# caterer-z-t/GRiD

Measured on AMD Instinct MI355X. Metric: samples/sec end-to-end steps 4–7 (50k×3M bins); k-NN distance HBM GB/s vs peak, higher is better.
Workload: dtype f64 (statistics) + bf16-MFMA exact-integer (k-NN)

## Files before the change

grid_amd/_abi.py:

```python
from __future__ import annotations

import ctypes as C
import os
import sys
from pathlib import Path

import numpy as np

_HERE = Path(__file__).resolve().parent
LIB_PATH = Path(os.environ.get("GRID_AMD_LIB", _HERE / "_lib" / "libgridhip.so"))

GRID_OK, GRID_EINVAL, GRID_EHIP, GRID_EZERODIV, GRID_EUNSUPPORTED, GRID_ERANGE = range(6)
MISSING = -(2 ** 31)
ZQ_NAN = -(2 ** 31)
ZQ_NEG0 = -(2 ** 31) + 1
ZQ16_NAN, ZQ16_NEG0, ZQ16_ESC = -32768, -32767, -32766
BLOCK = 8192
KBW = 32
SEG_K1 = 16
SEL_STATE = 16
SEL_NVALID, SEL_RLOC, SEL_RTOT, SEL_NV, SEL_RUSE, SEL_ERR = 0, 1, 2, 3, 4, 5
SEL_THR, SEL_V0, SEL_SMIN, SEL_SMAX = 8, 9, 12, 13

_i64, _i32, _f64, _vp = C.c_int64, C.c_int32, C.c_double, C.c_void_p
# ... 122 lines not shown
    "grid_md_parse_map": [_vp, _vp, _vp, _vp, _i64, _vp, _vp, _vp, _vp, _vp, _vp, _i64, _vp, _i64, _vp, _i64, _vp,
                          _vp, _vp],
    "grid_md_parse_ref_general": [_vp, _vp, _vp, _vp, _i64, _vp, _vp, _vp, _vp, _vp, _i64, _vp, _vp, _vp, _vp,
                                  C.POINTER(_i64)],
    "grid_md_parse_map_general": [_vp, _vp, _vp, _vp, _i64, _vp, _vp, _vp, _vp, _vp, _vp, _i64, _vp, _i64, _vp, _i64,
                                  _vp, _vp, _vp],
    "grid_fill_i32": [_vp, _vp, _i64, _i32],
    "grid_md_finish": [_vp, _vp, _i64, _i64, _i64, _vp, _i32, _f64, _f64, _vp, _vp, _vp, _vp, _vp, C.POINTER(_i64)],
    "grid_md_gather": [_vp, _vp, _i64, _i64, _i64, _vp, _vp, _vp, _vp, _i64, _vp, _vp, _vp],
    "grid_ctx_own_stream_cumask": [_vp, _vp, _i32],
    "grid_ctx_stream": [_vp, C.POINTER(_vp)],
    "grid_knn_seg_pack": [_vp, _vp, _i64, _i64, _i64, _vp],
    "grid_knn_seg_tiles_pack": [_vp, _vp, _i64, _i64, _i64, _i64, _vp],
    "grid_knn_seg_rows_fill": [_vp, _vp, _i64, _vp, _i64, _i64, _i64, _vp, _i64],
    "grid_md_popsum": [_vp, _vp, _i64, _i64, _vp, _i32, _vp, _vp],
    "grid_md_popvalid": [_vp, _vp, _vp, _i64, _f64, _f64, _vp],
    "grid_md_rowstats": [_vp, _vp, _i64, _i64, _i64, _vp, _vp, _vp, _vp, C.POINTER(_i64)],
    "grid_md_pack_shards": [_vp, _vp, _i64, _i64, _vp, _vp, _vp, _i32, _vp, _i32, _vp],
    "grid_gz_parts_new": [C.POINTER(_vp)],
    "grid_gz_parts_header": [_vp, _i64, _i64, _vp, _vp, _i32, _i32],
    "grid_gz_parts_rows": [_vp, _i64, _i64, _i64, C.c_char_p, _vp, _vp, _i64, _i32, _i32],
    "grid_gz_parts_rows_dev": [_vp, _vp, _i64, _i64, _i64, C.c_char_p, _vp, _vp, _i64, _i32, _i64],
    "grid_gz_parts_size": [_vp, C.POINTER(_i64)],
    "grid_gz_parts_write": [_vp, C.c_char_p, _i64, _i32],
    "grid_gz_parts_free": [_vp],
    "grid_ntext_count": [_vp, _vp, _vp, _vp, _i64, _vp, _vp, _vp, _i64, _vp, _vp, _vp, _vp, _vp, _vp],
    "grid_ntext_parse": [_vp, _vp, _vp, _vp, _vp, _i64, _vp, _vp, _vp, _i64, _i64, _vp, _i64, _vp, _vp, _vp],
    "grid_ntext_prefix": [_vp, _vp, _i64, _vp, _i64, _vp],
    "grid_ntext_parse_host": [_vp, _i64, _i64, _i64, _i64, _vp, _i64, _vp, _i64, C.POINTER(_i32), C.POINTER(_i64)],
    "grid_ntext_rows_host": [_vp, _i64, _vp, _i64, C.POINTER(_i64), _vp, _vp],
    "grid_ntext_index_open": [C.c_char_p, _i32, C.POINTER(_vp), C.POINTER(_i64), C.POINTER(_i64), C.POINTER(_i64)],
    "grid_ntext_index_fetch": [_vp, _vp, _vp, _vp, _vp, _vp, _vp],
    "grid_ntext_index_free": [_vp],
}
EXPORTS = tuple(_SIGS) + ("grid_last_error", "grid_build_info")


class GridNativeError(RuntimeError):

    def __init__(self, msg, code=None):
        super().__init__(msg)
        self.code = code


_lib = None


def load():
    global _lib
    if _lib is not None:
        return _lib
    if not LIB_PATH.exists():
        raise GridNativeError(f"{LIB_PATH} not built: run `python -c 'import __graft_entry__ as g; g.build()'` "
                              "or `make -C grid_amd/csrc`")
    lib = C.CDLL(str(LIB_PATH), mode=C.RTLD_GLOBAL)
    try:
        for name, args in _SIGS.items():
            f = getattr(lib, name)
            f.argtypes = args
            f.restype = C.c_int
        lib.grid_last_error.argtypes = []
        lib.grid_last_error.restype = C.c_char_p
        info = _build_info(lib)
    except AttributeError as e:
        raise GridNativeError(f"{LIB_PATH} lacks an entry point this package binds ({e}): rebuild with "
                              "`make -C grid_amd/csrc`") from None
    files = info.get("src_files")
    if files and (_CSRC / "Makefile").exists():
        named = sorted(n for n in files.split() if not n.startswith(".."))
        if named != _HASHED:
            raise GridNativeError(f"{LIB_PATH} hashed other source files ({' '.join(named)}) than this tree "
                                  f"lists: rebuild with `make -C grid_amd/csrc`")
    want = source_sha256(files.split() if files else None)
    if want is not None and info.get("src_sha256") != want:
        raise GridNativeError(f"{LIB_PATH} was built from other sources (library {info.get('src_sha256')}, "
                              f"tree {want}): rebuild with `make -C grid_amd/csrc`")
    _lib = lib
    return lib


_CSRC = _HERE / "csrc"
_HASHED = sorted(["core.hip", "normalize.hip", "knn.hip", "dipcn_phase.hip", "synth.hip", "depth16.hip",
                  "inflate.hip", "mosdepth_dev.hip", "gzwrite.hip", "ntext_dev.hip", "ingest.cpp", "textio.cpp",
                  "hapnbr.cpp", "common.hpp", "synth_model.hpp", "inflate_core.hpp", "ntext_core.hpp", "fastgz.hpp"])


def source_sha256(names=None):
    import hashlib
    if names is not None:
        files = [_CSRC / f for f in names]
    else:
        files = [_CSRC / f for f in _HASHED] + [_HERE.parent / "include" / "grid_abi.h"]
    if not all(f.exists() for f in files):
        return None
    h = hashlib.sha256()
    for f in files:
        h.update(f.read_bytes())
    return h.hexdigest()


def _build_info(lib):
    import json
    lib.grid_build_info.argtypes = [C.c_char_p, C.c_int64]
    lib.grid_build_info.restype = C.c_int
    buf = C.create_string_buffer(512)
    lib.grid_build_info(buf, 512)
    return json.loads(buf.value.decode())


def build_info():
    return _build_info(load())


def check(rc: int, what: str = ""):
    if rc == GRID_OK:
        return
    msg = load().grid_last_error().decode(errors="replace")
    if rc == GRID_EZERODIV:
        raise ZeroDivisionError(msg or "float division by zero")
    raise GridNativeError(f"{what}: {msg} (code {rc})", rc)


def call(name: str, *args):
    check(getattr(load(), name)(*args), name)


def ptr(a) -> int:
    if a is None:
        return None
    if isinstance(a, np.ndarray):
        if not a.flags.c_contiguous:
            raise ValueError("array must be C-contiguous")
        return a.ctypes.data
    if isinstance(a, DevBuf):
        return a.ptr
    if hasattr(a, "data_ptr"):
        return a.data_ptr()
    return int(a)


class PinnedBuf:

    def __init__(self, nbytes: int):
        h = _vp()
        call("grid_host_alloc", int(nbytes), C.byref(h))
        self.ptr, self.nbytes = h.value, int(nbytes)
        self.array = np.ctypeslib.as_array((C.c_uint8 * self.nbytes).from_address(self.ptr))

    def free(self):
        if self.ptr:
            self.array = None
            load().grid_host_free(self.ptr)
            self.ptr = 0

    def __del__(self):
        try:
            self.free()
        except Exception:
            pass


class Device:

    def __init__(self, device: int = 0, stream=None):
        lib = load()
        self.index = device
        h = _vp()
# ... 572 lines not shown
```

grid_amd/csrc/mosdepth_dev.hip:

```cpp
#include "common.hpp"

#include <hipcub/hipcub.hpp>

#include <algorithm>

namespace {

constexpr int CH = 16384, SEG = 64, PTH = CH / SEG, MAXLINE = 256;

struct MdOpts {
  const char *prefix;
  int npre;
  int has_window;
  int64_t wstart, wend;
  int nmask;
  const char *mnames;
  const int32_t *mname_off;
  const int64_t *mkb_off;
  const int64_t *mkb;
};

template <class P>
__device__ __forceinline__ bool md_masked(const MdOpts &o, P c, int clen, int64_t s, int64_t e) {
  if (o.nmask == 0) return false;
  const bool has = clen >= 3 && c[0] == 'c' && c[1] == 'h' && c[2] == 'r';
  const int nlen = has ? clen : clen + 3;
  for (int k = 0; k < o.nmask; k++) {
    const int a = o.mname_off[k], b = o.mname_off[k + 1];
    if (b - a != nlen) continue;
    bool eq = true;
    for (int t = 0; t < nlen && eq; t++) {
      const char want = o.mnames[a + t];
      const char got = has ? (char)c[t] : (t < 3 ? "chr"[t] : (char)c[t - 3]);
      eq = want == got;
    }
    if (!eq) continue;
    const int64_t lo = s >= 0 ? s / 1000 : -((-s + 999) / 1000);
    const int64_t hi = e >= 0 ? e / 1000 : -((-e + 999) / 1000);
    if (hi < lo) return false;
    int64_t l = o.mkb_off[k], r = o.mkb_off[k + 1];
    while (l < r) {
      const int64_t m = (l + r) >> 1;
      if (o.mkb[m] < lo) l = m + 1;
      else r = m;
    }
    return l < o.mkb_off[k + 1] && o.mkb[l] <= hi;
  }
  return false;
}

__device__ __forceinline__ uint32_t nl_bits(uint32_t w) {
  const uint32_t x = w ^ 0x0A0A0A0Au;
  return ~(((x & 0x7F7F7F7Fu) + 0x7F7F7F7Fu) | x | 0x7F7F7F7Fu);
}

__global__ __launch_bounds__(256) void k_md_count(const uint8_t *__restrict__ text, const int64_t *__restrict__ toff,
                                                  const int64_t *__restrict__ tlen, const int32_t *__restrict__ cfile,
                                                  const int64_t *__restrict__ cstart, int32_t *__restrict__ cnl,
                                                  int32_t *__restrict__ flags, const int32_t *__restrict__ fst) {
  const int c = blockIdx.x, f = cfile[c];
  if (fst && fst[f]) return;
  const int64_t a = cstart[c], b = min(tlen[f], a + CH);
  const uint8_t *t = text + toff[f];
  int n = 0, hi = 0;
  for (int64_t i = a + threadIdx.x * 16; i < b; i += 256 * 16) {
    if (i + 16 <= b) {
      const uint4 v = *reinterpret_cast<const uint4 *>(t + i);
      n += __builtin_popcount(nl_bits(v.x)) + __builtin_popcount(nl_bits(v.y)) + __builtin_popcount(nl_bits(v.z)) +
           __builtin_popcount(nl_bits(v.w));
      hi |= ((v.x | v.y | v.z | v.w) & 0x80808080u) != 0;
    } else {
      for (int64_t j = i; j < b; j++) {
        n += t[j] == '\n';
        hi |= t[j] >= 0x80;
      }
    }
  }
  for (int o = 32; o > 0; o >>= 1) {
    n += __shfl_xor(n, o, 64);
    hi |= __shfl_xor(hi, o, 64);
  }
  __shared__ int s_n[4], s_hi[4];
  if ((threadIdx.x & 63) == 0) {
// ... 7 lines not shown
  }
}

__global__ __launch_bounds__(256) void k_md_scan(const int32_t *__restrict__ cfirst, const int32_t *__restrict__ cnl,
                                                 int64_t *__restrict__ cline0, int nfiles) {
  __shared__ int64_t s_w[4];
  const int f = blockIdx.x, tid = threadIdx.x, lane = tid & 63, wv = tid >> 6;
  if (f >= nfiles) return;
  const int c0 = cfirst[f], c1 = cfirst[f + 1];
  int64_t base = 0;
  for (int r = c0; r < c1; r += 256) {
    const int c = r + tid;
    const int64_t v = c < c1 ? cnl[c] : 0;
    int64_t incl = v;
#pragma unroll
    for (int d = 1; d < 64; d <<= 1) {
      const int64_t y = __shfl_up(incl, d, 64);
      if (lane >= d) incl += y;
    }
    if (lane == 63) s_w[wv] = incl;
    __syncthreads();
    int64_t before = base;
    for (int w = 0; w < wv; w++) before += s_w[w];
    if (c < c1) cline0[c] = before + incl - v;
    base += s_w[0] + s_w[1] + s_w[2] + s_w[3];
    __syncthreads();
  }
}

template <class P>
__device__ __forceinline__ bool md_line(P p, int len, int &clen, int64_t &s, int64_t &e, int64_t &q) {
  int i = 0;
  while (i < len && (unsigned)(p[i] - 0x21) < 0x5e) i++;
  if (i == 0 || i == len || p[i] != '\t') return false;
  clen = i++;
  int64_t v[2];
  for (int k = 0; k < 2; k++) {
    const int d = i;
    int64_t x = 0;
    while (i < len && (unsigned)(p[i] - '0') < 10) x = x * 10 + (p[i++] - '0');
    if (i == d || i - d > 18 || i == len || p[i] != '\t') return false;
    v[k] = x;
    i++;
  }
  const int d = i;
  int64_t ip = 0;
  while (i < len && (unsigned)(p[i] - '0') < 10) ip = ip * 10 + (p[i++] - '0');
  if (i == d || i - d > 15) return false;
  int64_t fp = 0;
  if (i < len) {
    if (p[i] != '.') return false;
    i++;
    const int f0 = i;
    while (i < len && (unsigned)(p[i] - '0') < 10) fp = fp * 10 + (p[i++] - '0');
    if (i != len || i - f0 > 2) return false;
    if (i - f0 == 1) fp *= 10;
  }
  q = ip * 100 + fp;
  if (q > 2147483647LL) return false;
  s = v[0];
  e = v[1];
  return true;
}

struct Key2 {
  int64_t s, e;
};

__device__ __forceinline__ bool key_lt(int64_t as, int64_t ae, const Key2 &b) {
  return as < b.s || (as == b.s && ae < b.e);
}

__device__ __forceinline__ uint32_t nl_mask16(const uint4 v) {
  const uint32_t w[4] = {v.x, v.y, v.z, v.w};
  uint32_t m = 0;
#pragma unroll
  for (int k = 0; k < 4; k++) {
    const uint32_t z = nl_bits(w[k]);
    m |= (((z >> 7) & 1u) | ((z >> 14) & 2u) | ((z >> 21) & 4u) | ((z >> 28) & 8u)) << (4 * k);
  }
  return m;
}

__device__ __forceinline__ int md_phys(int i) { return i + 4 * ((i + 48) >> 6); }
struct PadText {
  const uint8_t *t;
  int i0;
  __device__ __forceinline__ uint8_t operator[](int k) const { return t[md_phys(i0 + k)]; }
};

constexpr int64_t MD_TAG_MAXLINE = 0x7fffffffLL - 3;
__device__ __forceinline__ int32_t md_tag(int64_t idx) { return (int32_t)(GRID_MISSING + 1 + (int32_t)idx); }

#ifndef GRID_MDPARSE_WPE
#define GRID_MDPARSE_WPE 8
#endif
#ifndef GRID_MDPARSE_G
#define GRID_MDPARSE_G 3
#endif
template <int MODE>
__global__ __launch_bounds__(PTH) __attribute__((amdgpu_waves_per_eu(GRID_MDPARSE_WPE))) void k_md_parse(const uint8_t *__restrict__ text, const int64_t *__restrict__ toff,
                                                  const int64_t *__restrict__ tlen,
                                                  const int32_t *__restrict__ cfile,
                                                  const int64_t *__restrict__ cstart,
                                                  const int64_t *__restrict__ cline0, MdOpts o,
                                                  int32_t *__restrict__ flags,
                                                  uint8_t *__restrict__ ref_kept, Key2 *__restrict__ ref_keys,
                                                  int64_t ref_cap,
                                                  const Key2 *__restrict__ K, int64_t nK,
                                                  const int32_t *__restrict__ ref_kidx, int64_t ref_nlines,
                                                  int32_t *__restrict__ Q, int64_t ldq,
                                                  const int32_t *__restrict__ qrow,
                                                  unsigned long long *__restrict__ kept,
                                                  const int32_t *__restrict__ fst) {
  constexpr int HALO = 16, SPAN = HALO + CH + MAXLINE + 16;
  static_assert(HALO == 16 && SEG == 64, "md_phys: block t + 1 = segment t");
  __shared__ __attribute__((aligned(16))) uint8_t s_t[SPAN + 4 * (SPAN / 64 + 2)];
  __shared__ int s_wsum[PTH / 64];
  const int c = blockIdx.x, f = cfile[c], tid = threadIdx.x;
  if (fst && fst[f]) return;
  const int64_t L = tlen[f], a = cstart[c], b = min(L, a + CH);
  const uint8_t *t = text + toff[f];
  {
    const int64_t lo = a - HALO, hi = min(L, b + MAXLINE);
    constexpr int NW = SPAN / 16, G = GRID_MDPARSE_G;
    for (int k0 = 0; k0 * PTH < NW; k0 += G) {
      uint4 v[G];
#pragma unroll
      for (int k = 0; k < G; k++) {
        const int w = tid + (k0 + k) * PTH;
        const int64_t p = lo + 16 * (int64_t)w;
        v[k] = make_uint4(0, 0, 0, 0);
        if (w < NW && p >= 0 && p + 16 <= hi) v[k] = *reinterpret_cast<const uint4 *>(t + p);
      }
#pragma unroll
      for (int k = 0; k < G; k++) {
        const int w = tid + (k0 + k) * PTH;
        const int64_t p = lo + 16 * (int64_t)w;
        if (w >= NW) continue;
        if (p >= 0 && p + 16 > hi && p < hi) {
          uint8_t q[16];
          for (int j = 0; j < 16; j++) q[j] = p + j < hi ? t[p + j] : 0;
          v[k] = *reinterpret_cast<const uint4 *>(q);
        }
        uint32_t *d = reinterpret_cast<uint32_t *>(s_t + md_phys(16 * w));
        d[0] = v[k].x;
        d[1] = v[k].y;
        d[2] = v[k].z;
        d[3] = v[k].w;
      }
    }
  }
  __syncthreads();
  const int64_t s0 = a + (int64_t)tid * SEG, s1 = min(b, s0 + SEG);
  const int nw = s1 > s0 ? (int)((s1 - s0 + 15) / 16) : 0;
  const uint32_t *seg = reinterpret_cast<const uint32_t *>(s_t + md_phys(HALO + tid * SEG));
  auto mask = [&](int k) {
    uint32_t mk = nl_mask16(make_uint4(seg[4 * k], seg[4 * k + 1], seg[4 * k + 2], seg[4 * k + 3]));
    const int64_t rest = s1 - (s0 + 16 * k);
    if (rest < 16) mk &= (1u << rest) - 1u;
    return mk;
  };
  int nl = 0;
  for (int k = 0; k < nw; k++) nl += __builtin_popcount(mask(k));
  int incl = nl;
#pragma unroll
  for (int d = 1; d < 64; d <<= 1) {
    const int y = __shfl_up(incl, d, 64);
    if ((tid & 63) >= d) incl += y;
  }
  if ((tid & 63) == 63) s_wsum[tid >> 6] = incl;
  __syncthreads();
  int before = incl - nl;
  for (int w = 0; w < (tid >> 6); w++) before += s_wsum[w];
  const int64_t idx0 = cline0[c] + before;
  int bad = 0;
  unsigned long long nkept = 0;
  auto line = [&](int64_t x, int len, int64_t idx) {
    const PadText p{s_t, (int)(HALO + (x - a))};
    if (o.npre != 0) {
      if (len < o.npre) return;
      for (int k = 0; k < o.npre; k++)
        if (p[k] != (uint8_t)o.prefix[k]) return;
    }
    int clen;
    int64_t s, e, q;
    if (!md_line(p, len, clen, s, e, q)) {
      bad |= GRID_MD_EXOTIC;
      return;
    }
    if (!((MODE == 0 || q > 0) && (!o.has_window || (e >= o.wstart && s <= o.wend)) &&
          !md_masked(o, p, clen, s, e)))
      return;
    if (MODE == 0) {
      if (idx < ref_cap) {
        ref_kept[idx] = 1;
        ref_keys[idx] = Key2{s, e};
      } else {
        bad |= GRID_MD_NOTINK;
      }
    } else {
      int64_t j = idx < ref_nlines ? ref_kidx[idx] : -1;
      if (j < 0 || K[j].s != s || K[j].e != e) {
        int64_t l = 0, r = nK;
        while (l < r) {
          const int64_t mid = (l + r) >> 1;
          if (K[mid].s < s || (K[mid].s == s && K[mid].e < e)) l = mid + 1;
          else r = mid;
        }
        j = (l < nK && K[l].s == s && K[l].e == e) ? l : -1;
      }
      if (j < 0) {
        bad |= GRID_MD_NOTINK;
      } else if (MODE == 1) {
        Q[(int64_t)qrow[f] * ldq + j] = (int32_t)q;
        nkept++;
      } else if (idx > MD_TAG_MAXLINE) {
        bad |= GRID_MD_LINES;
      } else {
        int32_t *cell = Q + (int64_t)qrow[f] * ldq + j;
        const int32_t tag = md_tag(idx);
        if (MODE == 2) {
          atomicMax(cell, tag);
        } else if (*cell == tag) {
          *cell = (int32_t)q;
          nkept++;
        }
      }
    }
  };
  if (s1 > s0) {
    int64_t cur = (s0 == 0 || s_t[md_phys((int)(HALO + (s0 - a) - 1))] == '\n') ? s0 : -1;
    int64_t idx = idx0;
    for (int k = 0; k < nw; k++) {
      uint32_t mk = mask(k);
      while (mk) {
        const int64_t y = s0 + 16 * k + __builtin_ctz(mk);
        mk &= mk - 1;
        if (cur >= 0) {
          const int64_t len = y - cur;
          if (len > MAXLINE) bad |= GRID_MD_EXOTIC;
          else line(cur, (int)len, idx);
        }
        idx++;
        cur = y + 1 < s1 ? y + 1 : -1;
      }
    }
    if (cur >= 0) {
      const PadText p{s_t, (int)(HALO + (cur - a))};
      const int64_t lim = min(L, cur + MAXLINE + 1) - cur;
      int len = 0;
      while (len < lim && p[len] != '\n') len++;
      if (len > MAXLINE) bad |= GRID_MD_EXOTIC;
      else line(cur, len, idx);
    }
  }
  if (bad) atomicOr(flags + f, bad);
  if (MODE == 1 || MODE == 3) {
    for (int k = 32; k > 0; k >>= 1) nkept += __shfl_xor(nkept, k, 64);
    if ((tid & 63) == 0 && nkept) atomicAdd(kept + f, nkept);
  }
}

__global__ void k_file_status(const int32_t *__restrict__ ust, const int64_t *__restrict__ owner, int64_t n,
                              int32_t *__restrict__ fst) {
  const int64_t u = (int64_t)blockIdx.x * blockDim.x + threadIdx.x;
  if (u < n && ust[u] != 0) atomicOr(fst + owner[u], 1);
}

__global__ void k_md_ref_index(const uint8_t *__restrict__ kept, const int64_t *__restrict__ pos, int64_t n,
                               const Key2 *__restrict__ keys, Key2 *__restrict__ K, int32_t *__restrict__ kidx) {
  const int64_t i = (int64_t)blockIdx.x * blockDim.x + threadIdx.x;
  if (i >= n) return;
  if (kept[i]) {
    K[pos[i]] = keys[i];
    kidx[i] = (int32_t)pos[i];
  } else {
    kidx[i] = -1;
  }
}

__global__ void k_md_sorted(const Key2 *__restrict__ K, int64_t nK, int32_t *__restrict__ bad) {
  const int64_t j = (int64_t)blockIdx.x * blockDim.x + threadIdx.x;
  if (j + 1 >= nK) return;
  if (!key_lt(K[j].s, K[j].e, K[j + 1])) atomicOr(bad, 1);
}

__global__ void k_md_gk_pack(const uint8_t *__restrict__ kept, const int64_t *__restrict__ pos, int64_t n,
                             const Key2 *__restrict__ keys, int64_t *__restrict__ ps, int64_t *__restrict__ pe,
                             int32_t *__restrict__ pline, int32_t *__restrict__ iota, int32_t *__restrict__ kidx) {
  const int64_t i = (int64_t)blockIdx.x * blockDim.x + threadIdx.x;
  if (i >= n) return;
  kidx[i] = -1;
  if (kept[i]) {
    const int64_t p = pos[i];
    ps[p] = keys[i].s;
    pe[p] = keys[i].e;
    pline[p] = (int32_t)i;
    iota[p] = (int32_t)p;
  }
}

__global__ void k_md_gk_take(const int64_t *__restrict__ src, const int32_t *__restrict__ perm, int64_t n,
                             int64_t *__restrict__ dst) {
  const int64_t i = (int64_t)blockIdx.x * blockDim.x + threadIdx.x;
  if (i < n) dst[i] = src[perm[i]];
}

__global__ void k_md_gk_heads(const int64_t *__restrict__ ss, const int64_t *__restrict__ pe,
                              const int32_t *__restrict__ perm, int64_t n, int32_t *__restrict__ head) {
  const int64_t i = (int64_t)blockIdx.x * blockDim.x + threadIdx.x;
  if (i >= n) return;
  head[i] = i == 0 || ss[i] != ss[i - 1] || pe[perm[i]] != pe[perm[i - 1]];
}

__global__ void k_md_gk_index(const int64_t *__restrict__ ss, const int64_t *__restrict__ pe,
                              const int32_t *__restrict__ perm, const int32_t *__restrict__ pline,
                              const int32_t *__restrict__ head, const int64_t *__restrict__ hpos, int64_t n,
                              Key2 *__restrict__ K, int32_t *__restrict__ kidx) {
  const int64_t i = (int64_t)blockIdx.x * blockDim.x + threadIdx.x;
  if (i >= n) return;
  const int32_t r = perm[i];
  const int64_t rank = hpos[i] + head[i] - 1;
  if (head[i]) K[rank] = Key2{ss[i], pe[r]};
  kidx[pline[r]] = (int32_t)rank;
}

__global__ void k_fill_i32(int32_t *__restrict__ p, int64_t n, int32_t v) {
  for (int64_t i = (int64_t)blockIdx.x * blockDim.x + threadIdx.x; i < n; i += (int64_t)gridDim.x * blockDim.x)
    p[i] = v;
}

__global__ __launch_bounds__(256) void k_md_popmeans(const int32_t *__restrict__ Q, int64_t ldq, int64_t nK,
                                                     const int32_t *__restrict__ rows, int nrows, double min_d,
                                                     double max_d, double *__restrict__ mean,
                                                     int32_t *__restrict__ valid) {
  const int64_t j = (int64_t)blockIdx.x * blockDim.x + threadIdx.x;
// ... 71 lines not shown
                                                     unsigned long long *__restrict__ present,
                                                     unsigned long long *__restrict__ nvalid) {
  const int r = blockIdx.y;
  unsigned long long a = 0, v = 0;
  for (int64_t j = (int64_t)blockIdx.x * blockDim.x + threadIdx.x; j < nK; j += (int64_t)gridDim.x * blockDim.x) {
    const bool p = Q[(int64_t)r * ldq + j] != GRID_MISSING;
    a += p;
    v += p && valid[j];
  }
  for (int o = 32; o > 0; o >>= 1) {
    a += __shfl_xor(a, o, 64);
    v += __shfl_xor(v, o, 64);
  }
  if ((threadIdx.x & 63) == 0) {
    if (a) atomicAdd(present + r, a);
    if (v) atomicAdd(nvalid + r, v);
  }
}

__global__ __launch_bounds__(256) void k_md_gather(const int32_t *__restrict__ Q, int64_t ldq, int64_t nK,
                                                   const int32_t *__restrict__ valid,
                                                   const int64_t *__restrict__ cpos,
                                                   const int32_t *__restrict__ dst_row, int32_t *__restrict__ out,
                                                   int64_t ldo) {
  const int r = blockIdx.y;
  const int32_t d = dst_row[r];
  if (d < 0) return;
  for (int64_t j = (int64_t)blockIdx.x * blockDim.x + threadIdx.x; j < nK; j += (int64_t)gridDim.x * blockDim.x)
    if (valid[j]) out[(int64_t)d * ldo + cpos[j]] = Q[(int64_t)r * ldq + j];
}

__global__ void k_md_cols(const Key2 *__restrict__ K, int64_t nK, const int32_t *__restrict__ valid,
                          const int64_t *__restrict__ cpos, int64_t *__restrict__ starts, int64_t *__restrict__ ends) {
  const int64_t j = (int64_t)blockIdx.x * blockDim.x + threadIdx.x;
  if (j < nK && valid[j]) {
    starts[cpos[j]] = K[j].s;
    ends[cpos[j]] = K[j].e;
  }
}

template <class T>
struct ToI64 {
  __host__ __device__ __forceinline__ int64_t operator()(const T &v) const { return (int64_t)v; }
};

template <class TI>
int excl_scan(grid_ctx *ctx, const TI *in, int64_t *out, int64_t n) {
  REQUIRE(n < (1ll << 31), "scan too long");
  hipcub::TransformInputIterator<int64_t, ToI64<TI>, const TI *> it(in, ToI64<TI>());
  size_t tmp = 0;
  HIPCHK(hipcub::DeviceScan::ExclusiveScan(nullptr, tmp, it, out, hipcub::Sum(), (int64_t)0, (int)n, ctx->stream));
  void *s = nullptr;
  int rc = grid_scratch(ctx, tmp + 256, &s);
  if (rc) return rc;
  HIPCHK(hipcub::DeviceScan::ExclusiveScan(s, tmp, it, out, hipcub::Sum(), (int64_t)0, (int)n, ctx->stream));
  return GRID_OK;
}

struct CovLoci {
  int nchrom, nloci;
  const char *names;
  const int32_t *name_off;
  const int32_t *lfirst;
  const int64_t *maxlen;
  const int64_t *ls, *le;
  const int32_t *lid;
};
constexpr int64_t COV_MAXBP = 1ll << 62, COV_MAXLINE = 0xffffffffll;

__global__ __launch_bounds__(PTH) __attribute__((amdgpu_waves_per_eu(GRID_MDPARSE_WPE))) void k_md_cover(
    const uint8_t *__restrict__ text, const int64_t *__restrict__ toff, const int64_t *__restrict__ tlen,
    const int32_t *__restrict__ cfile, const int64_t *__restrict__ cstart, const int64_t *__restrict__ cline0,
    CovLoci T, int32_t *__restrict__ flags, const int32_t *__restrict__ fst, unsigned long long *__restrict__ cursor,
    unsigned long long cap, uint64_t *__restrict__ hkey, int64_t *__restrict__ hov, int32_t *__restrict__ hq) {
  constexpr int HALO = 16, SPAN = HALO + CH + MAXLINE + 16;
  __shared__ __attribute__((aligned(16))) uint8_t s_t[SPAN + 4 * (SPAN / 64 + 2)];
  __shared__ int s_wsum[PTH / 64];
  const int c = blockIdx.x, f = cfile[c], tid = threadIdx.x;
  if (fst && fst[f]) return;
  const int64_t L = tlen[f], a = cstart[c], b = min(L, a + CH);
  const uint8_t *t = text + toff[f];
  {
    const int64_t lo = a - HALO, hi = min(L, b + MAXLINE);
    constexpr int NW = SPAN / 16, G = GRID_MDPARSE_G;
    for (int k0 = 0; k0 * PTH < NW; k0 += G) {
      uint4 v[G];
#pragma unroll
      for (int k = 0; k < G; k++) {
        const int w = tid + (k0 + k) * PTH;
        const int64_t p = lo + 16 * (int64_t)w;
        v[k] = make_uint4(0, 0, 0, 0);
        if (w < NW && p >= 0 && p + 16 <= hi) v[k] = *reinterpret_cast<const uint4 *>(t + p);
      }
#pragma unroll
      for (int k = 0; k < G; k++) {
        const int w = tid + (k0 + k) * PTH;
        const int64_t p = lo + 16 * (int64_t)w;
        if (w >= NW) continue;
        if (p >= 0 && p + 16 > hi && p < hi) {
          uint8_t q[16];
          for (int j = 0; j < 16; j++) q[j] = p + j < hi ? t[p + j] : 0;
          v[k] = *reinterpret_cast<const uint4 *>(q);
        }
        uint32_t *d = reinterpret_cast<uint32_t *>(s_t + md_phys(16 * w));
        d[0] = v[k].x;
        d[1] = v[k].y;
        d[2] = v[k].z;
        d[3] = v[k].w;
      }
    }
  }
  __syncthreads();
  const int64_t s0 = a + (int64_t)tid * SEG, s1 = min(b, s0 + SEG);
  const int nw = s1 > s0 ? (int)((s1 - s0 + 15) / 16) : 0;
  const uint32_t *seg = reinterpret_cast<const uint32_t *>(s_t + md_phys(HALO + tid * SEG));
  auto mask = [&](int k) {
    uint32_t mk = nl_mask16(make_uint4(seg[4 * k], seg[4 * k + 1], seg[4 * k + 2], seg[4 * k + 3]));
    const int64_t rest = s1 - (s0 + 16 * k);
    if (rest < 16) mk &= (1u << rest) - 1u;
    return mk;
  };
  int nl = 0;
  for (int k = 0; k < nw; k++) nl += __builtin_popcount(mask(k));
  int incl = nl;
#pragma unroll
  for (int d = 1; d < 64; d <<= 1) {
    const int y = __shfl_up(incl, d, 64);
    if ((tid & 63) >= d) incl += y;
  }
  if ((tid & 63) == 63) s_wsum[tid >> 6] = incl;
  __syncthreads();
  int before = incl - nl;
  for (int w = 0; w < (tid >> 6); w++) before += s_wsum[w];
  const int64_t idx0 = cline0[c] + before;
  int bad = 0;
  auto line = [&](int64_t x, int len, int64_t idx) {
    const PadText p{s_t, (int)(HALO + (x - a))};
    int clen;
    int64_t s, e, q;
    if (!md_line(p, len, clen, s, e, q)) {
      bad |= GRID_MD_EXOTIC;
      return;
    }
    int lo = 0, hi = T.nchrom, ch = -1;
    while (lo < hi) {
      const int mid = (lo + hi) >> 1, n0 = T.name_off[mid];
      int cmp = clen - (T.name_off[mid + 1] - n0);
      for (int k = 0; cmp == 0 && k < clen; k++) cmp = (int)p[k] - (int)(uint8_t)T.names[n0 + k];
      if (cmp == 0) {
        ch = mid;
        break;
      }
      if (cmp < 0) hi = mid;
      else lo = mid + 1;
    }
    if (ch < 0) return;
    const int l0 = T.lfirst[ch];
    int l = l0, r = T.lfirst[ch + 1];
    while (l < r) {
      const int m = (l + r) >> 1;
      if (T.ls[m] < e) l = m + 1;
      else r = m;
    }
    const int64_t low = s - T.maxlen[ch];
    for (int j = l - 1; j >= l0 && T.ls[j] > low; j--) {
      const int64_t ov = min(T.le[j], e) - max(T.ls[j], s);
      if (ov <= 0) continue;
// ... 444 lines not shown
```

Before: 415.3.

## Parse mosdepth lines via shared-memory character-class bitmaps and SWAR digit conversion

```diff
diff --git a/grid_amd/_abi.py b/grid_amd/_abi.py
--- a/grid_amd/_abi.py
+++ b/grid_amd/_abi.py
@@ -228,7 +228,8 @@
 _CSRC = _HERE / "csrc"
 _HASHED = sorted(["core.hip", "normalize.hip", "knn.hip", "dipcn_phase.hip", "synth.hip", "depth16.hip",
                   "inflate.hip", "mosdepth_dev.hip", "gzwrite.hip", "ntext_dev.hip", "ingest.cpp", "textio.cpp",
-                  "hapnbr.cpp", "common.hpp", "synth_model.hpp", "inflate_core.hpp", "ntext_core.hpp", "fastgz.hpp"])
+                  "hapnbr.cpp", "common.hpp", "synth_model.hpp", "inflate_core.hpp", "ntext_core.hpp",
+                  "mdline_core.hpp", "fastgz.hpp"])
 
 
 def source_sha256(names=None):
diff --git a/grid_amd/csrc/mdline_core.hpp b/grid_amd/csrc/mdline_core.hpp
--- /dev/null
+++ b/grid_amd/csrc/mdline_core.hpp
@@ -0,0 +1,167 @@
+#pragma once
+#include <cstdint>
+
+#if defined(__HIPCC__)
+#define MDL_HD __host__ __device__ __forceinline__
+#else
+#define MDL_HD inline
+#endif
+
+namespace mdl {
+
+constexpr int FAST_MAXLEN = 63;
+enum { NL = 0, CHROM = 1, DIGIT = 2, SEP = 3, NCLASS = 4 };
+
+MDL_HD int md_phys(int i) { return i + 4 * ((i + 48) >> 6); }
+
+MDL_HD int ctz64(uint64_t x) { return x ? __builtin_ctzll(x) : 64; }
+MDL_HD int popc64(uint64_t x) { return __builtin_popcountll(x); }
+
+MDL_HD uint32_t perm(uint32_t hi, uint32_t lo, uint32_t sel) {
+#if defined(__HIP_DEVICE_COMPILE__)
+  return __builtin_amdgcn_perm(hi, lo, sel);
+#else
+  const uint64_t v = ((uint64_t)hi << 32) | lo;
+  uint32_t r = 0;
+  for (int k = 0; k < 4; k++) r |= (uint32_t)((v >> (8 * ((sel >> (8 * k)) & 7))) & 0xff) << (8 * k);
+  return r;
+#endif
+}
+
+MDL_HD uint32_t pack_nibbles(uint32_t u) {
+  const uint32_t t = u | (u >> 4);
+  return (t & 0xffu) | ((t >> 8) & 0xff00u);
+}
+
+struct Cls {
+  uint32_t m[NCLASS];
+};
+
+MDL_HD Cls class_masks(uint32_t w0, uint32_t w1, uint32_t w2, uint32_t w3) {
+  const uint32_t t0 = perm(w1, w0, 0x05010400u), t1 = perm(w1, w0, 0x07030602u);
+  const uint32_t t2 = perm(w3, w2, 0x05010400u), t3 = perm(w3, w2, 0x07030602u);
+  const uint32_t r[4] = {perm(t2, t0, 0x05040100u), perm(t2, t0, 0x07060302u), perm(t3, t1, 0x05040100u),
+                         perm(t3, t1, 0x07060302u)};
+  uint32_t u[NCLASS] = {0, 0, 0, 0};
+#if defined(__HIP_DEVICE_COMPILE__)
+#pragma unroll
+#endif
+  for (int k = 0; k < 4; k++) {
+    const uint32_t lo = r[k] & 0x7f7f7f7fu, hm = ~r[k] & 0x80808080u;
+    const uint32_t nl = ~((lo ^ 0x0a0a0a0au) + 0x7f7f7f7fu) & hm;
+    const uint32_t ch = (lo + 0x5f5f5f5fu) & ~(lo + 0x01010101u) & hm;
+    const uint32_t dg = (lo + 0x50505050u) & ~(lo + 0x46464646u) & hm;
+    const uint32_t sp = ~(((lo ^ 0x09090909u) + 0x7f7f7f7fu) & ((lo ^ 0x2e2e2e2eu) + 0x7f7f7f7fu)) & hm;
+    u[NL] |= nl >> (7 - k);
+    u[CHROM] |= ch >> (7 - k);
+    u[DIGIT] |= dg >> (7 - k);
+    u[SEP] |= sp >> (7 - k);
+  }
+  Cls c;
+  for (int j = 0; j < NCLASS; j++) c.m[j] = pack_nibbles(u[j]);
+  return c;
+}
+
+struct Span {
+  const uint8_t *t;
+  const uint32_t *bm;
+  int bmw;
+};
+
+MDL_HD uint64_t window(const uint32_t *bm, int i) {
+  const int k = i >> 5, sh = i & 31;
+  const uint32_t b0 = bm[k], b1 = bm[k + 1], b2 = bm[k + 2];
+  const uint32_t lo = (uint32_t)((((uint64_t)b1 << 32) | b0) >> sh);
+  const uint32_t hi = (uint32_t)((((uint64_t)b2 << 32) | b1) >> sh);
+  return ((uint64_t)hi << 32) | lo;
+}
+MDL_HD uint64_t window(const Span &s, int cls, int i) { return window(s.bm + cls * s.bmw, i); }
+
+MDL_HD uint32_t dword(const uint8_t *t, int j) { return *reinterpret_cast<const uint32_t *>(t + md_phys(j)); }
+
+MDL_HD void fetch8(const uint8_t *t, int e, uint32_t &lo, uint32_t &hi) {
+  const int p = e - 8, j = p & ~3, sh = 8 * (p & 3);
+  const uint32_t w0 = dword(t, j), w1 = dword(t, j + 4), w2 = dword(t, j + 8);
+  lo = (uint32_t)((((uint64_t)w1 << 32) | w0) >> sh);
+  hi = (uint32_t)((((uint64_t)w2 << 32) | w1) >> sh);
+}
+
+MDL_HD uint32_t conv4(uint32_t w) {
+  const uint32_t t = w * 10u + (w >> 8);
+  return (t & 0xffu) * 100u + ((t >> 16) & 0xffu);
+}
+MDL_HD uint32_t conv8(uint32_t lo, uint32_t hi) { return conv4(lo) * 10000u + conv4(hi); }
+
+MDL_HD void keep_digits(uint32_t &lo, uint32_t &hi, int n) {
+  const uint64_t m = n > 0 ? 0x0f0f0f0f0f0f0f0full << (8 * (8 - n)) : 0;
+  lo &= (uint32_t)m;
+  hi &= (uint32_t)(m >> 32);
+}
+
+MDL_HD uint64_t number(const uint8_t *t, int e, int d) {
+  uint32_t lo, hi;
+  fetch8(t, e, lo, hi);
+  keep_digits(lo, hi, d < 8 ? d : 8);
+  uint64_t v = conv8(lo, hi);
+  if (d > 8) {
+    fetch8(t, e - 8, lo, hi);
+    keep_digits(lo, hi, d - 8);
+    v += (uint64_t)conv8(lo, hi) * 100000000ull;
+  }
+  return v;
+}
+
+MDL_HD uint32_t fraction(const uint8_t *t, int e, int nf) {
+  const int p = e - 2, j = p & ~3, sh = 8 * (p & 3);
+  const uint32_t w0 = dword(t, j), w1 = dword(t, j + 4);
+  const uint32_t v = (uint32_t)((((uint64_t)w1 << 32) | w0) >> sh);
+  const uint32_t a = v & 0xfu, b = (v >> 8) & 0xfu;
+  return nf == 2 ? a * 10u + b : nf == 1 ? b * 10u : 0u;
+}
+
+MDL_HD bool starts_with8(const uint8_t *t, int i, uint64_t pw, int n) {
+  uint32_t lo, hi;
+  fetch8(t, i + 8, lo, hi);
+  const uint64_t v = ((uint64_t)hi << 32) | lo;
+  const uint64_t m = n >= 8 ? ~0ull : (1ull << (8 * n)) - 1;
+  return (v & m) == pw;
+}
+
+MDL_HD int line_len(const Span &sp, int i, int64_t lim) {
+  const int n = ctz64(window(sp, NL, i));
+  return n <= lim ? n : (int)lim;
+}
+
+struct Rec {
+  int clen;
+  int64_t s, e, q;
+};
+
+MDL_HD bool fast_line(const Span &sp, int i, int len, Rec &r) {
+  const uint64_t lm = (1ull << len) - 1;
+  const uint64_t cw = window(sp, CHROM, i) & lm, dw = window(sp, DIGIT, i) & lm, sw = window(sp, SEP, i) & lm;
+  const uint64_t tw = sw & ~cw;
+  if (popc64(tw) != 3) return false;
+  const uint64_t tw2 = tw & (tw - 1);
+  const int t1 = ctz64(tw), t2 = ctz64(tw2), t3 = ctz64(tw2 & (tw2 - 1));
+  if (t1 == 0 || ctz64(~cw) != t1) return false;
+  const uint64_t x = lm & ~((2ull << t1) - 1) & ~dw & ~tw;
+  if (x & (x - 1)) return false;
+  int pe = len, nf = 0;
+  if (x) {
+    if (!(x & sw)) return false;
+    pe = ctz64(x);
+    nf = len - pe - 1;
+  }
+  const int d1 = t2 - t1 - 1, d2 = t3 - t2 - 1, d3 = pe - t3 - 1;
+  if (d1 < 1 || d1 > 16 || d2 < 1 || d2 > 16 || d3 < 1 || d3 > 15 || nf > 2) return false;
+  const int64_t q = (int64_t)number(sp.t, i + pe, d3) * 100 + fraction(sp.t, i + len, nf);
+  if (q > 2147483647LL) return false;
+  r.clen = t1;
+  r.s = (int64_t)number(sp.t, i + t2, d1);
+  r.e = (int64_t)number(sp.t, i + t3, d2);
+  r.q = q;
+  return true;
+}
+
+}
diff --git a/grid_amd/csrc/mosdepth_dev.hip b/grid_amd/csrc/mosdepth_dev.hip
--- a/grid_amd/csrc/mosdepth_dev.hip
+++ b/grid_amd/csrc/mosdepth_dev.hip
@@ -1,4 +1,5 @@
 #include "common.hpp"
+#include "mdline_core.hpp"
 
 #include <hipcub/hipcub.hpp>
 
@@ -172,7 +173,7 @@
   return m;
 }
 
-__device__ __forceinline__ int md_phys(int i) { return i + 4 * ((i + 48) >> 6); }
+__device__ __forceinline__ int md_phys(int i) { return mdl::md_phys(i); }
 struct PadText {
   const uint8_t *t;
   int i0;
@@ -189,7 +190,7 @@
 #define GRID_MDPARSE_G 3
 #endif
 template <int MODE>
-__global__ __launch_bounds__(PTH) __attribute__((amdgpu_waves_per_eu(GRID_MDPARSE_WPE))) void k_md_parse(const uint8_t *__restrict__ text, const int64_t *__restrict__ toff,
+__global__ __launch_bounds__(PTH) __attribute__((amdgpu_waves_per_eu(6))) void k_md_parse(const uint8_t *__restrict__ text, const int64_t *__restrict__ toff,
                                                   const int64_t *__restrict__ tlen,
                                                   const int32_t *__restrict__ cfile,
                                                   const int64_t *__restrict__ cstart,
@@ -206,6 +207,10 @@
   constexpr int HALO = 16, SPAN = HALO + CH + MAXLINE + 16;
   static_assert(HALO == 16 && SEG == 64, "md_phys: block t + 1 = segment t");
   __shared__ __attribute__((aligned(16))) uint8_t s_t[SPAN + 4 * (SPAN / 64 + 2)];
+  constexpr int BMW = (SPAN / 16 + 1) / 2 + 1;
+  static_assert(((HALO + CH - 1) >> 5) + 2 < SPAN / 32, "window reads stay inside the bitmap that is written");
+  static_assert(HALO + CH - 1 + MAXLINE + 8 + 3 < SPAN, "word reads stay inside the span");
+  __shared__ uint32_t s_bm[mdl::NCLASS * BMW];
   __shared__ int s_wsum[PTH / 64];
   const int c = blockIdx.x, f = cfile[c], tid = threadIdx.x;
   if (fst && fst[f]) return;
@@ -238,21 +243,23 @@
         d[1] = v[k].y;
         d[2] = v[k].z;
         d[3] = v[k].w;
+        const mdl::Cls cm = mdl::class_masks(v[k].x, v[k].y, v[k].z, v[k].w);
+#pragma unroll
+        for (int j = 0; j < mdl::NCLASS; j++) reinterpret_cast<uint16_t *>(s_bm + j * BMW)[w] = (uint16_t)cm.m[j];
       }
     }
   }
   __syncthreads();
+  const mdl::Span sp{s_t, s_bm, BMW};
   const int64_t s0 = a + (int64_t)tid * SEG, s1 = min(b, s0 + SEG);
-  const int nw = s1 > s0 ? (int)((s1 - s0 + 15) / 16) : 0;
-  const uint32_t *seg = reinterpret_cast<const uint32_t *>(s_t + md_phys(HALO + tid * SEG));
-  auto mask = [&](int k) {
-    uint32_t mk = nl_mask16(make_uint4(seg[4 * k], seg[4 * k + 1], seg[4 * k + 2], seg[4 * k + 3]));
-    const int64_t rest = s1 - (s0 + 16 * k);
-    if (rest < 16) mk &= (1u << rest) - 1u;
-    return mk;
-  };
-  int nl = 0;
-  for (int k = 0; k < nw; k++) nl += __builtin_popcount(mask(k));
+  const int i0 = HALO + tid * SEG;
+  uint64_t nls = 0, starts = 0;
+  if (s1 > s0) {
+    const uint64_t in = s1 - s0 >= 64 ? ~0ull : (1ull << (s1 - s0)) - 1;
+    nls = mdl::window(sp, mdl::NL, i0) & in;
+    starts = (mdl::window(sp, mdl::NL, i0 - 1) | (uint64_t)(s0 == 0)) & in;
+  }
+  const int nl = mdl::popc64(nls);
   int incl = nl;
 #pragma unroll
   for (int d = 1; d < 64; d <<= 1) {
@@ -264,24 +271,54 @@
   int before = incl - nl;
   for (int w = 0; w < (tid >> 6); w++) before += s_wsum[w];
   const int64_t idx0 = cline0[c] + before;
+  uint64_t pw0 = 0;
+  for (int k = 0; k < min(o.npre, 8); k++) pw0 |= (uint64_t)(uint8_t)o.prefix[k] << (8 * k);
   int bad = 0;
   unsigned long long nkept = 0;
-  auto line = [&](int64_t x, int len, int64_t idx) {
-    const PadText p{s_t, (int)(HALO + (x - a))};
+  while (starts) {
+    const int k0 = mdl::ctz64(starts);
+    starts &= starts - 1;
+    const int64_t x = s0 + k0, idx = idx0 + mdl::popc64(nls & ((1ull << k0) - 1));
+    const int i = i0 + k0;
+    const PadText p{s_t, i};
+    int len = mdl::line_len(sp, i, L - x);
+    const bool shortline = len <= mdl::FAST_MAXLEN;
+    if (!shortline) {
+      const int64_t lim = min(L, x + MAXLINE + 1) - x;
+      len = 0;
+      while (len < lim && p[len] != '\n') len++;
+      if (len > MAXLINE) {
+        bad |= GRID_MD_EXOTIC;
+        continue;
+      }
+    }
     if (o.npre != 0) {
-      if (len < o.npre) return;
-      for (int k = 0; k < o.npre; k++)
-        if (p[k] != (uint8_t)o.prefix[k]) return;
+      if (len < o.npre) continue;
+      if (!mdl::starts_with8(s_t, i, pw0, min(o.npre, 8))) continue;
+      bool eq = true;
+      for (int k = 8; k < o.npre && eq; k += 8) {
+        uint64_t pw = 0;
+        const int n = min(o.npre - k, 8);
+        for (int j = 0; j < n; j++) pw |= (uint64_t)(uint8_t)o.prefix[k + j] << (8 * j);
+        eq = mdl::starts_with8(s_t, i + k, pw, n);
+      }
+      if (!eq) continue;
     }
     int clen;
     int64_t s, e, q;
-    if (!md_line(p, len, clen, s, e, q)) {
+    mdl::Rec rec;
+    if (shortline && mdl::fast_line(sp, i, len, rec)) {
+      clen = rec.clen;
+      s = rec.s;
+      e = rec.e;
+      q = rec.q;
+    } else if (!md_line(p, len, clen, s, e, q)) {
       bad |= GRID_MD_EXOTIC;
-      return;
+      continue;
     }
     if (!((MODE == 0 || q > 0) && (!o.has_window || (e >= o.wstart && s <= o.wend)) &&
           !md_masked(o, p, clen, s, e)))
-      return;
+      continue;
     if (MODE == 0) {
       if (idx < ref_cap) {
         ref_kept[idx] = 1;
@@ -317,32 +354,6 @@
           nkept++;
         }
       }
-    }
-  };
-  if (s1 > s0) {
-    int64_t cur = (s0 == 0 || s_t[md_phys((int)(HALO + (s0 - a) - 1))] == '\n') ? s0 : -1;
-    int64_t idx = idx0;
-    for (int k = 0; k < nw; k++) {
-      uint32_t mk = mask(k);
-      while (mk) {
-        const int64_t y = s0 + 16 * k + __builtin_ctz(mk);
-        mk &= mk - 1;
-        if (cur >= 0) {
-          const int64_t len = y - cur;
-          if (len > MAXLINE) bad |= GRID_MD_EXOTIC;
-          else line(cur, (int)len, idx);
-        }
-        idx++;
-        cur = y + 1 < s1 ? y + 1 : -1;
-      }
-    }
-    if (cur >= 0) {
-      const PadText p{s_t, (int)(HALO + (cur - a))};
-      const int64_t lim = min(L, cur + MAXLINE + 1) - cur;
-      int len = 0;
-      while (len < lim && p[len] != '\n') len++;
-      if (len > MAXLINE) bad |= GRID_MD_EXOTIC;
-      else line(cur, len, idx);
     }
   }
   if (bad) atomicOr(flags + f, bad);
```

Result: no change. 422.9, median of 6 (+1.8%).

## Parse mosdepth lines one-per-thread via shared line-start table instead of per-segment scans

Applied to the files above, without the earlier changes.

```diff
diff --git a/grid_amd/csrc/mosdepth_dev.hip b/grid_amd/csrc/mosdepth_dev.hip
--- a/grid_amd/csrc/mosdepth_dev.hip
+++ b/grid_amd/csrc/mosdepth_dev.hip
@@ -185,9 +185,7 @@
 #ifndef GRID_MDPARSE_WPE
 #define GRID_MDPARSE_WPE 8
 #endif
-#ifndef GRID_MDPARSE_G
-#define GRID_MDPARSE_G 3
-#endif
+constexpr int MD_WIN = 1024;
 template <int MODE>
 __global__ __launch_bounds__(PTH) __attribute__((amdgpu_waves_per_eu(GRID_MDPARSE_WPE))) void k_md_parse(const uint8_t *__restrict__ text, const int64_t *__restrict__ toff,
                                                   const int64_t *__restrict__ tlen,
@@ -204,8 +202,9 @@
                                                   unsigned long long *__restrict__ kept,
                                                   const int32_t *__restrict__ fst) {
   constexpr int HALO = 16, SPAN = HALO + CH + MAXLINE + 16;
-  static_assert(HALO == 16 && SEG == 64, "md_phys: block t + 1 = segment t");
-  __shared__ __attribute__((aligned(16))) uint8_t s_t[SPAN + 4 * (SPAN / 64 + 2)];
+  static_assert(SEG == 64 && CH <= 0xffff, "a segment is one 64-bit newline mask; starts fit 16 bits");
+  __shared__ __attribute__((aligned(16))) uint8_t s_t[SPAN];
+  __shared__ uint16_t s_st[MD_WIN + 2];
   __shared__ int s_wsum[PTH / 64];
   const int c = blockIdx.x, f = cfile[c], tid = threadIdx.x;
   if (fst && fst[f]) return;
@@ -213,7 +212,7 @@
   const uint8_t *t = text + toff[f];
   {
     const int64_t lo = a - HALO, hi = min(L, b + MAXLINE);
-    constexpr int NW = SPAN / 16, G = GRID_MDPARSE_G;
+    constexpr int NW = SPAN / 16, G = 3;
     for (int k0 = 0; k0 * PTH < NW; k0 += G) {
       uint4 v[G];
 #pragma unroll
@@ -233,26 +232,23 @@
           for (int j = 0; j < 16; j++) q[j] = p + j < hi ? t[p + j] : 0;
           v[k] = *reinterpret_cast<const uint4 *>(q);
         }
-        uint32_t *d = reinterpret_cast<uint32_t *>(s_t + md_phys(16 * w));
-        d[0] = v[k].x;
-        d[1] = v[k].y;
-        d[2] = v[k].z;
-        d[3] = v[k].w;
+        *reinterpret_cast<uint4 *>(s_t + 16 * w) = v[k];
       }
     }
   }
   __syncthreads();
-  const int64_t s0 = a + (int64_t)tid * SEG, s1 = min(b, s0 + SEG);
-  const int nw = s1 > s0 ? (int)((s1 - s0 + 15) / 16) : 0;
-  const uint32_t *seg = reinterpret_cast<const uint32_t *>(s_t + md_phys(HALO + tid * SEG));
-  auto mask = [&](int k) {
-    uint32_t mk = nl_mask16(make_uint4(seg[4 * k], seg[4 * k + 1], seg[4 * k + 2], seg[4 * k + 3]));
-    const int64_t rest = s1 - (s0 + 16 * k);
-    if (rest < 16) mk &= (1u << rest) - 1u;
-    return mk;
-  };
-  int nl = 0;
-  for (int k = 0; k < nw; k++) nl += __builtin_popcount(mask(k));
+  const int blen = (int)(b - a), o0 = tid * SEG;
+  uint64_t nlm = 0;
+  if (o0 < blen) {
+    const uint4 *seg = reinterpret_cast<const uint4 *>(s_t + HALO + o0);
+#pragma unroll
+    for (int k = 0; k < 4; k++) {
+      const int kk = (k + (tid >> 2)) & 3;
+      nlm |= (uint64_t)nl_mask16(seg[kk]) << (16 * kk);
+    }
+    if (blen - o0 < SEG) nlm &= (1ull << (blen - o0)) - 1ull;
+  }
+  const int nl = __builtin_popcountll(nlm);
   int incl = nl;
 #pragma unroll
   for (int d = 1; d < 64; d <<= 1) {
@@ -261,13 +257,15 @@
   }
   if ((tid & 63) == 63) s_wsum[tid >> 6] = incl;
   __syncthreads();
-  int before = incl - nl;
-  for (int w = 0; w < (tid >> 6); w++) before += s_wsum[w];
-  const int64_t idx0 = cline0[c] + before;
+  int before = incl - nl, nnl = 0;
+  for (int w = 0; w < PTH / 64; w++) {
+    if (w < (tid >> 6)) before += s_wsum[w];
+    nnl += s_wsum[w];
+  }
+  const int64_t idx0 = cline0[c];
   int bad = 0;
   unsigned long long nkept = 0;
-  auto line = [&](int64_t x, int len, int64_t idx) {
-    const PadText p{s_t, (int)(HALO + (x - a))};
+  auto line = [&](const uint8_t *p, int len, int64_t idx) {
     if (o.npre != 0) {
       if (len < o.npre) return;
       for (int k = 0; k < o.npre; k++)
@@ -319,30 +317,31 @@
       }
     }
   };
-  if (s1 > s0) {
-    int64_t cur = (s0 == 0 || s_t[md_phys((int)(HALO + (s0 - a) - 1))] == '\n') ? s0 : -1;
-    int64_t idx = idx0;
-    for (int k = 0; k < nw; k++) {
-      uint32_t mk = mask(k);
-      while (mk) {
-        const int64_t y = s0 + 16 * k + __builtin_ctz(mk);
-        mk &= mk - 1;
-        if (cur >= 0) {
-          const int64_t len = y - cur;
-          if (len > MAXLINE) bad |= GRID_MD_EXOTIC;
-          else line(cur, (int)len, idx);
-        }
-        idx++;
-        cur = y + 1 < s1 ? y + 1 : -1;
-      }
-    }
-    if (cur >= 0) {
-      const PadText p{s_t, (int)(HALO + (cur - a))};
-      const int64_t lim = min(L, cur + MAXLINE + 1) - cur;
+  const bool own0 = a == 0 || s_t[HALO - 1] == '\n';
+  for (int w0 = 0; w0 <= nnl; w0 += MD_WIN) {
+    if (w0) __syncthreads();
+    if (w0 == 0 && tid == 0) s_st[0] = 0;
+    {
+      int k = before + 1 - w0;
+      for (uint64_t m = nlm; m && k <= MD_WIN; m &= m - 1, k++)
+        if (k >= 0) s_st[k] = (uint16_t)(o0 + __builtin_ctzll(m) + 1);
+    }
+    __syncthreads();
+    const int rend = min(w0 + MD_WIN, nnl + 1);
+    for (int r = w0 + tid; r < rend; r += PTH) {
+      const int st = s_st[r - w0];
+      const uint8_t *p = s_t + HALO + st;
+      bool own = r > 0 || own0;
       int len = 0;
-      while (len < lim && p[len] != '\n') len++;
+      if (r < nnl) {
+        len = s_st[r - w0 + 1] - 1 - st;
+      } else if ((own = own && st < blen)) {
+        const int lim = (int)min(L - (a + st), (int64_t)MAXLINE + 1);
+        while (len < lim && p[len] != '\n') len++;
+      }
+      if (!own) continue;
       if (len > MAXLINE) bad |= GRID_MD_EXOTIC;
-      else line(cur, len, idx);
+      else line(p, len, idx0 + r);
     }
   }
   if (bad) atomicOr(flags + f, bad);
@@ -580,7 +579,7 @@
   const uint8_t *t = text + toff[f];
   {
     const int64_t lo = a - HALO, hi = min(L, b + MAXLINE);
-    constexpr int NW = SPAN / 16, G = GRID_MDPARSE_G;
+    constexpr int NW = SPAN / 16, G = 3;
     for (int k0 = 0; k0 * PTH < NW; k0 += G) {
       uint4 v[G];
 #pragma unroll
```

Measured after the change: 414.2 before, 418.1 after, median of 4. About the same (+0.9%).
